# cage-challenge/cage-challenge-4

Hardware: AMD Instinct MI355X
Metric: agent-env steps/sec (5 blue agents x N envs) (higher is better)
Workload: dtype int32

## Files before the change

### cage_challenge_4_amd/csrc/cc4_engine.h

```cpp
#pragma once
#include "cc4_state.h"
#include "cc4_tables.h"

namespace cc4 {

struct Ctx { EnvState* s; EnvCold* c; Rng* r; HostDyn* hd; StepWork* w; unsigned long long* prof = nullptr;
             unsigned long long* aprof = nullptr; EvLog* lg = nullptr; const uint64_t* gpre = nullptr;
             const ExtAct* ext = nullptr; };

#if defined(__HIP_DEVICE_COMPILE__)
#define CC4_TICK(x, i) do { if ((x).prof) { unsigned long long _t = clock64(); (x).prof[(i)] += _t - (x).prof[15]; (x).prof[15] = _t; } } while (0)
#define CC4_TICK0(x) do { if ((x).prof) (x).prof[15] = clock64(); } while (0)
#define CC4_AT0(x) unsigned long long _at = (x).aprof ? clock64() : 0
#define CC4_AT(x, k) do { if ((x).aprof) { unsigned long long _n = clock64(); (x).aprof[(k)] += _n - _at; _at = _n; } } while (0)
#if defined(CC4_FINE)
#define CC4_FT0(x, r) unsigned long long _ft = ((x).aprof && (r) == 0) ? clock64() : 0
#define CC4_FT(x, r, k) do { if ((x).aprof && (r) == 0) { unsigned long long _n = clock64(); (x).aprof[88 + (k)] += _n - _ft; _ft = _n; } } while (0)
#else
#define CC4_FT0(x, r) do { } while (0)
#define CC4_FT(x, r, k) do { } while (0)
#endif
#else
#define CC4_FT0(x, r) do { } while (0)
#define CC4_FT(x, r, k) do { } while (0)
// ... 344 lines not shown
  return r;
}
CC4_HD int rs_kth_on_host(const EnvState* s, const RedAgent& a, int h, int kth) {
  const int n = a.h.nsess;
  for (int i0 = 0; i0 < n; i0 += 8) {
    const S8 q = rs_load8(s, a, i0);
    int hit = -1;
    CC4_UNROLL for (int k = 0; k < 8; ++k)
      if (hit < 0 && i0 + k < n && rsw_host(q.v[k]) == h) { if (kth == 0) hit = i0 + k; kth--; }
    if (hit >= 0) return hit;
  }
  return -1;
}
CC4_HD int rs_find_host_pid(const EnvState* s, const RedAgent& a, int h, int pid) {
  const int n = a.h.nsess;
  for (int i0 = 0; i0 < n; i0 += 8) {
    const S8 q = rs_load8(s, a, i0);
    int hit = -1;
    CC4_UNROLL for (int k = 7; k >= 0; --k) if (i0 + k < n && rsw_host(q.v[k]) == h && rsw_pid(q.v[k]) == pid) hit = i0 + k;
    if (hit >= 0) return hit;
  }
  return -1;
}
struct RedPre { int si = -1; HostSess hs = {0, -1, -1}; bool ok = false; };
#if defined(__HIPCC__)
__device__ __forceinline__ RedPre rs_wave_query(const EnvState* s, int lane, int sid, int host) {
  const int r = lane >> 3, k = lane & 7, ra = r < NRED ? r : 0;
  const RedAgent& A = s->red[ra];
  const int ksid = __builtin_amdgcn_ds_bpermute(ra << 2, sid), khost = __builtin_amdgcn_ds_bpermute(ra << 2, host);
  const int n = (r < NRED && ksid >= 0) ? (int)A.h.nsess : 0;
  const int sh = 8 * k;
  RedPre p; p.ok = true;
  for (int i0 = 0; __ballot(i0 < n); i0 += 8) {
    const bool v = i0 + k < n;
    uint64_t w = 0;
    if (v) w = rs_word(s, A.sord[i0 + k]);
    const bool on = v && rsw_host(w) == khost;
    const uint32_t bid = (uint32_t)(__ballot(v && rsw_id(w) == ksid) >> sh) & 0xFFu;
    const uint32_t bh = (uint32_t)(__ballot(on) >> sh) & 0xFFu, br = (uint32_t)(__ballot(on && (rsw_flags(w) & RS_ROOT)) >> sh) & 0xFFu;
    if (p.si < 0 && bid) p.si = i0 + ctz32(bid);
    p.hs.n += __popc(bh);
    if (p.hs.first < 0 && bh) p.hs.first = i0 + ctz32(bh);
    if (p.hs.first_root < 0 && br) p.hs.first_root = i0 + ctz32(br);
  }
  return p;
}
#endif
CC4_HD void rs_list_remove(RedAgent& a, int idx) {
  uint64_t w[MAX_RS / 8];
  __builtin_memcpy(w, a.sord, MAX_RS);
  const int wi = idx >> 3, sh = 8 * (idx & 7);
  CC4_UNROLL for (int k = 0; k < MAX_RS / 8; ++k) {
    if (k < wi) continue;
    const uint64_t nxt = k + 1 < MAX_RS / 8 ? w[k + 1] : 0ull;
    uint64_t v = (w[k] >> 8) | (nxt << 56);
    if (k == wi && sh) v = (w[k] & ((1ull << sh) - 1ull)) | (v & ~((1ull << sh) - 1ull));
    w[k] = v;
  }
  __builtin_memcpy(a.sord, w, MAX_RS);
}
CC4_HD int rs_alloc_lowest(Ctx x) {
  for (int w = 0; w < RS_POOL / 32; ++w) {
    const uint32_t fr = ~x.s->spool_used[w];
    if (fr) return w * 32 + ctz32(fr);
  }
  return -1;
}
CC4_HD void rs_reserve(Ctx x) {
  uint32_t used[RS_POOL / 32];
  CC4_UNROLL for (int w = 0; w < RS_POOL / 32; ++w) used[w] = x.s->spool_used[w];
  int ty[NRED];
  CC4_UNROLL for (int r = 0; r < NRED; ++r) ty[r] = x.s->rexec[r].type;
  CC4_UNROLL for (int r = 0; r < NRED; ++r) {
    int slot = 0xFF;
    if (ty[r] == RA_EXPLOIT) {
      CC4_UNROLL for (int w = 0; w < RS_POOL / 32; ++w) {
        const uint32_t fr = ~used[w];
        if (slot == 0xFF && fr) { slot = w * 32 + ctz32(fr); used[w] |= 1u << (slot & 31); }
      }
    }
    x.w->rs_slot[r] = (uint8_t)slot;
  }
}
CC4_HD int rs_add(Ctx x, int r, int host, int pid, int flags, int slot = -1) {
  EnvState* s = x.s;
  RedAgent& a = s->red[r];
  if (slot < 0) slot = rs_alloc_lowest(x);
  if (a.h.nsess >= MAX_RS || slot < 0 || slot >= RS_POOL) { set_err(x, E_RSESS_OVERFLOW); return -1; }
  int id = 0;
  for (int i0 = 0; i0 < a.h.nsess; i0 += 8) {
    const S8 q = rs_load8(s, a, i0);
    CC4_UNROLL for (int k = 0; k < 8; ++k) if (i0 + k < a.h.nsess && rsw_id(q.v[k]) + 1 > id) id = rsw_id(q.v[k]) + 1;
  }
  (void)or_shared(&s->spool_used[slot >> 5], 1u << (slot & 31));
  rs_word_put(s, slot, rsw_make(id, pid, host, flags));
  if (flags & RS_ABSTRACT) {
    uint64_t* row = reinterpret_cast<uint64_t*>(x.c->kports[slot]);
    for (int k = 0; k < (MAXH + 7) / 8; ++k) row[k] = 0;
  }
  a.sord[a.h.nsess++] = (uint8_t)slot;
  a.h.rsc_dirty = 1; a.h.fsm_dirty = 1;
  if (!bit_get(a.live_hosts, host)) { bit_set(a.live_hosts, host); a.h.nlive++; }
  bit_set_shared(s->red_hosts, host);
  return a.h.nsess - 1;
}
CC4_HD void rs_host_left(Ctx x, int r, int gone) {
  RedAgent& a = x.s->red[r];
  bit_clr(a.live_hosts, gone); a.h.nlive--;
  uint32_t lw[NRED];
  CC4_UNROLL for (int q = 0; q < NRED; ++q) lw[q] = x.s->red[q].live_hosts[gone >> 5];
  uint32_t any_other = 0;
  CC4_UNROLL for (int q = 0; q < NRED; ++q) any_other |= lw[q];
  if (!((any_other >> (gone & 31)) & 1u)) bit_clr_shared(x.s->red_hosts, gone);
}
CC4_HD void rs_remove_at(Ctx x, int r, int idx, bool keep_record = false) {
  EnvState* s = x.s;
  RedAgent& a = s->red[r];
  const int slot = a.sord[idx];
  const int gone = rsw_host(rs_word(s, slot));
  if (!keep_record) bit_clr_shared(s->spool_used, slot);
  rs_list_remove(a, idx);
  a.h.nsess--;
  a.h.rsc_dirty = 1; a.h.fsm_dirty = 1;
  if (rs_on_host(s, a, gone).n == 0) rs_host_left(x, r, gone);
}
CC4_HD void rs_remove_on_host(Ctx x, int r, int h) {
  EnvState* s = x.s;
  RedAgent& a = s->red[r];
  const int n = a.h.nsess;
  int out = 0, removed = 0;
  bool left = false;
  for (int i0 = 0; i0 < n; i0 += 8) {
    const S8 q = rs_load8(s, a, i0);
    CC4_UNROLL for (int k = 0; k < 8; ++k) {
      if (i0 + k >= n) continue;
      const bool here = rsw_host(q.v[k]) == h;
      if (here && !(rsw_flags(q.v[k]) & RS_ORIG)) { bit_clr_shared(s->spool_used, s8_slot(q, k)); removed++; continue; }
      if (here) left = true;
      if (out != i0 + k) a.sord[out] = (uint8_t)s8_slot(q, k);
      out++;
    }
  }
  if (!removed) return;
  a.h.nsess = (uint8_t)out;
  a.h.rsc_dirty = 1; a.h.fsm_dirty = 1;
  if (!left) rs_host_left(x, r, h);
}
CC4_HD void rs_move_to_end(EnvState* s, RedAgent& a, int idx, int new_id) {
  const int slot = a.sord[idx];
  rs_list_remove(a, idx);
  a.sord[a.h.nsess - 1] = (uint8_t)slot;
  if (new_id >= 0) rs_word_put(s, slot, (rs_word(s, slot) & ~0xFFFFull) | (uint64_t)(new_id & 0xFFFF));
  a.h.rsc_dirty = 1;
}
CC4_HD bool sid_known(const RedAgent& a, const uint16_t* ks, int id, int nknown) {
  if (id < 256) return bit_get(a.known_bm, id);
  for (int i = 0; i < nknown; ++i) if (ks[i] == id) return true;
  return false;
}
CC4_HD void as_know_sid(Ctx x, int r, int id) {
  RedAgent& a = x.s->red[r];
  if (sid_known(a, x.c->known_sid[r], id, a.h.nknown)) return;
  if (a.h.nknown >= MAX_KS) { set_err(x, E_KS_OVERFLOW); return; }
  x.c->known_sid[r][a.h.nknown++] = (uint16_t)id;
  if (id < 256) bit_set(a.known_bm, id);
}
// ... 1258 lines not shown
    }
    if (!bit_get(A.fsm_known, h)) {
      fsm_set_state(A, h, H.fsm_step == 0 ? FS_U : FS_K);
      A.fsm_order[H.fsm_n++] = (uint8_t)h;
      bit_set(A.fsm_known, h);
    }
    if (hn) bit_set(A.fsm_hn, h);
  }
  CC4_AT(x, 4);
  if (H.rsc_listed) {
    const B5 live = b5_load(A.live_hosts), known = b5_load(A.fsm_known), hn = b5_load(A.fsm_hn);
    seen = b5_or(seen, live);
    if (b5_any(b5_andn(live, known)))
      for (int i = 0; i < H.nsess; ++i) {
        int h = rsw_host(rs_at(x.s, A, i));
        if (bit_get(A.fsm_known, h)) continue;
        fsm_set_state(A, h, H.fsm_step == 0 ? FS_U : FS_K);
        A.fsm_order[H.fsm_n++] = (uint8_t)h;
        bit_set(A.fsm_known, h);
      }
    b5_store(A.fsm_hn, b5_or(hn, live));
    H.fsm_dirty = 0;
  }
  CC4_AT(x, 5);
  {
    const B5 lost = b5_andn(b5_load(A.fsm_ur), seen);
    if (b5_any(lost))
      CC4_UNROLL for (int w = 0; w < 5; ++w) {
        uint32_t m = lost.w[w];
        while (m) { int b = ctz32(m); m &= m - 1; fsm_set_state(A, w * 32 + b, FS_KD); }
      }
  }
  CC4_AT(x, 6);
}
CC4_HD int fsm_choose_host_discovery(Ctx x, int r, RedHdr& H) {
  RedAgent& A = x.s->red[r];
  uint32_t order = 0; int nst = 0; uint32_t seen = 0;
  for (int i = 0; i < H.fsm_n && nst < 8; ++i) {
    int st = fsm_get(A, A.fsm_order[i]);
    if (!((seen >> st) & 1u)) { seen |= 1u << st; order |= (uint32_t)st << (4 * nst); nst++; }
  }
  int sum = 0;
  for (int k = 0; k < nst; ++k) { int st = (order >> (4 * k)) & 0xF; sum += st <= FS_SD ? 20 : (st <= FS_UD ? 10 : 0); }
  int chosen_state;
  if (sum > 0) {
    double mult = 1.0 / ((double)sum / 100.0);
    double last = 0.0;
    for (int k = 0; k < nst; ++k) { int st = (order >> (4 * k)) & 0xF; int p = st <= FS_SD ? 20 : (st <= FS_UD ? 10 : 0); last = last + ((double)p / 100.0) * mult; }
    double u = rng_random(x.r);
    double run = 0.0; int idx = 0;
    for (int k = 0; k < nst; ++k) {
      int st = (order >> (4 * k)) & 0xF; int p = st <= FS_SD ? 20 : (st <= FS_UD ? 10 : 0);
      run = run + ((double)p / 100.0) * mult;
      if (run / last <= u) idx++;
    }
    if (idx >= nst) idx = nst - 1;
    chosen_state = (order >> (4 * idx)) & 0xF;
  } else {
    chosen_state = (order >> (4 * (int)rng_below(x.r, (uint32_t)nst))) & 0xF;
  }
  int n_all = 0, n_srv = 0;
  for (int i = 0; i < H.fsm_n; ++i) {
    int h = A.fsm_order[i];
    if (fsm_get(A, h) != chosen_state) continue;
    n_all++;
    if (h_is_server(h) && bit_get(A.fsm_hn, h)) n_srv++;
  }
  int want_srv = -1;
  if (n_all > 1 && n_srv > 0) {
    double i01 = rng_random(x.r);
    want_srv = (i01 <= 0.75 || n_srv == n_all) ? 1 : 0;
  }
  int cnt = want_srv < 0 ? n_all : (want_srv ? n_srv : n_all - n_srv);
  int c = (int)rng_below(x.r, (uint32_t)cnt);
  for (int i = 0; i < H.fsm_n; ++i) {
    int h = A.fsm_order[i];
    if (fsm_get(A, h) != chosen_state) continue;
    bool srv = h_is_server(h) && bit_get(A.fsm_hn, h);
    if (want_srv >= 0 && (int)srv != want_srv) continue;
    if (c-- == 0) return h;
  }
  return A.fsm_order[0];
}
CC4_HD Act fsm_get_action(Ctx x, int r, RedHdr& H, bool observed = false) {
  EnvState* s = x.s;
  RedAgent& A = s->red[r];
  Act out; out.type = RA_SLEEP; out.host = 0; out.arg = 0; out.ticks = 1; out.sid = 0; out.busy = 0;
  CC4_FT0(x, r);
  if (!observed) fsm_observe(x, r, H);
  CC4_FT(x, r, 5);
  if (H.obs_success == T_IN_PROGRESS) { H.fsm_step++; return out; }
  int n = H.fsm_n;
  if (n == 0) { set_err(x, E_FSM_NO_HOST); H.fsm_step++; return out; }
  const bool discovery = (s->policy & 3) == RP_DISCOVERY;
  int host;
  if (!discovery) host = A.fsm_order[rng_below(x.r, (uint32_t)n)];
  else host = fsm_choose_host_discovery(x, r, H);
  CC4_FT(x, r, 6);
  uint32_t pk;
  const int host_state = fsm_get(A, host);
  if (!discovery) switch (host_state) {
    case FS_K:  pk = 0xF432u << 16 | (RA_DRS | RA_AGGR << 4 | RA_STEALTH << 8); break;
    case FS_KD: pk = 0xFF42u << 16 | (RA_AGGR | RA_STEALTH << 4); break;
    case FS_S:  pk = 0xF431u << 16 | (RA_DRS | RA_EXPLOIT << 4 | RA_DECEPTION << 8); break;
    case FS_SD: pk = 0xFF43u << 16 | (RA_EXPLOIT | RA_DECEPTION << 4); break;
    case FS_U:  pk = 0xF442u << 16 | (RA_DRS | RA_PRIVESC << 4 | RA_WITHDRAW << 8); break;
    case FS_UD: pk = 0xFF44u << 16 | (RA_PRIVESC | RA_WITHDRAW << 4); break;
    case FS_R:  pk = 0x4432u << 16 | (RA_DRS | RA_DEGRADE << 4 | RA_IMPACT << 8 | RA_WITHDRAW << 12); break;
    default:    pk = 0xF442u << 16 | (RA_DEGRADE | RA_IMPACT << 4 | RA_WITHDRAW << 8); break;
  } else switch (host_state) {
    case FS_K:  pk = 0xF441u << 16 | (RA_DRS | RA_AGGR << 4 | RA_STEALTH << 8); break;
    case FS_KD: pk = 0xFF44u << 16 | (RA_AGGR | RA_STEALTH << 4); break;
    case FS_S:  pk = 0xF441u << 16 | (RA_DRS | RA_EXPLOIT << 4 | RA_DECEPTION << 8); break;
    case FS_SD: pk = 0xFF44u << 16 | (RA_EXPLOIT | RA_DECEPTION << 4); break;
    case FS_U:  pk = 0xF440u << 16 | (RA_DRS | RA_PRIVESC << 4 | RA_WITHDRAW << 8); break;
    case FS_UD: pk = 0xFF44u << 16 | (RA_PRIVESC | RA_WITHDRAW << 4); break;
    case FS_R:  pk = 0x4444u << 16 | (RA_DRS | RA_DEGRADE << 4 | RA_IMPACT << 8 | RA_WITHDRAW << 12); break;
    default:    pk = 0xF442u << 16 | (RA_DEGRADE | RA_IMPACT << 4 | RA_WITHDRAW << 8); break;
  }
  const int fl = rng_random_quarter(x.r);
  int k = 0;
  for (int i = 0; i < 4; ++i) if ((int)((pk >> (16 + 4 * i)) & 0xF) <= fl) k++;
  int t = (int)((pk >> (4 * k)) & 0xF);
  out.type = (uint8_t)t; out.host = (uint8_t)host;
  bool bad = false;
  if (t == RA_DRS) {
    uint32_t known = H.as_subnet;
    if (known == 0) bad = true; else out.arg = (uint8_t)nth_bit(known, (int)rng_below(x.r, (uint32_t)popc32(known)));
  }
  if ((t == RA_PRIVESC || t == RA_IMPACT || t == RA_DEGRADE) && !bit_get(A.fsm_hn, host)) bad = true;
  if (!bad) {
    if (H.nknown == 0) bad = true; else out.sid = x.c->known_sid[r][rng_below(x.r, (uint32_t)H.nknown)];
  }
  if (bad) { set_err(x, E_UNREACHABLE); out.type = RA_SLEEP; }
  out.ticks = (uint8_t)red_duration(out.type);
  H.fsm_step++;
  CC4_FT(x, r, 7);
  return out;
}
CC4_HD Act random_red_get_action(Ctx x, int r, RedHdr& H) {
  RedAgent& A = x.s->red[r];
  Act out; out.type = RA_SLEEP; out.host = 0; out.arg = 0; out.ticks = 1; out.sid = 0; out.busy = 0;
  const int nip = popc32(A.as_ip[0]) + popc32(A.as_ip[1]) + popc32(A.as_ip[2]) + popc32(A.as_ip[3]) + popc32(A.as_ip[4]);
  const int nhn = popc32(A.as_hn[0]) + popc32(A.as_hn[1]) + popc32(A.as_hn[2]) + popc32(A.as_hn[3]) + popc32(A.as_hn[4]);
  const int nsub = popc32(H.as_subnet), nsid = H.nknown;
  const uint8_t types[10] = {RA_DRS, RA_AGGR, RA_STEALTH, RA_EXPLOIT, RA_PRIVESC, RA_DEGRADE, RA_DECEPTION, RA_IMPACT, RA_WITHDRAW, RA_SLEEP};
  uint32_t valid = 0;
  for (int c = 0; c < 10; ++c) {
    int t = types[c];
    bool ok = true;
    if (t != RA_SLEEP && nsid == 0) ok = false;
    if (t == RA_DRS && nsub == 0) ok = false;
    if ((t == RA_AGGR || t == RA_STEALTH || t == RA_EXPLOIT || t == RA_DECEPTION || t == RA_WITHDRAW) && nip == 0) ok = false;
    if ((t == RA_PRIVESC || t == RA_DEGRADE || t == RA_IMPACT || t == RA_WITHDRAW) && nhn == 0) ok = false;
    if (ok) valid |= 1u << c;
  }
  const int t = types[nth_bit(valid, (int)rng_below(x.r, (uint32_t)popc32(valid)))];
  auto pick_sid = [&]() { return (int)x.c->known_sid[r][rng_below(x.r, (uint32_t)nsid)]; };
  auto pick_ip = [&]() { return nth_set(A.as_ip, 5, (int)rng_below(x.r, (uint32_t)nip)); };
  auto pick_hn = [&]() { return nth_set(A.as_hn, 5, (int)rng_below(x.r, (uint32_t)nhn)); };
  out.type = (uint8_t)t;
  switch (t) {
    case RA_DRS: out.arg = (uint8_t)nth_bit(H.as_subnet, (int)rng_below(x.r, (uint32_t)nsub)); out.sid = (uint16_t)pick_sid(); break;
    case RA_AGGR: case RA_STEALTH: case RA_DECEPTION: out.sid = (uint16_t)pick_sid(); out.host = (uint8_t)pick_ip(); break;
    case RA_EXPLOIT: out.host = (uint8_t)pick_ip(); out.sid = (uint16_t)pick_sid(); break;
    case RA_PRIVESC: case RA_DEGRADE: case RA_IMPACT: out.host = (uint8_t)pick_hn(); out.sid = (uint16_t)pick_sid(); break;
    case RA_WITHDRAW: out.sid = (uint16_t)pick_sid(); out.host = (uint8_t)pick_ip(); out.arg = (uint8_t)pick_hn(); break;
    default: break;
  }
  out.ticks = (uint8_t)red_duration(out.type);
  H.fsm_step++;
  return out;
}
CC4_HD void red_validate(Ctx x, int r, const RedHdr& H, Act& a) {
  RedAgent& A = x.s->red[r];
  if (a.type >= RA_SLEEP) return;
  bool ok = true;
  if (!sid_known(A, x.c->known_sid[r], a.sid, H.nknown)) ok = false;
  if (a.type == RA_DRS) { if (!((H.as_subnet >> a.arg) & 1u)) ok = false; }
  else if (a.type == RA_PRIVESC || a.type == RA_IMPACT || a.type == RA_DEGRADE) { if (!bit_get(A.as_hn, a.host)) ok = false; }
  else if (a.type == RA_WITHDRAW) { if (!bit_get(A.as_ip, a.host) || !bit_get(A.as_hn, a.arg)) ok = false; }
  else { if (!bit_get(A.as_ip, a.host)) ok = false; }
  if (!ok) { a.type = RA_INVALID; a.ticks = 1; }
}

CC4_HD constexpr uint32_t red_zone_hosts(int r, int w) {
  uint32_t m = 0;
  for (int i = 0; i < red_nsub(r); ++i) {
    int lo = red_subnet_alloc(r, i) * SLOTS - 32 * w, hi = lo + SLOTS - 1;
    if (hi < 0 || lo > 31) continue;
    uint32_t up = hi >= 31 ? 0xFFFFFFFFu : ((2u << hi) - 1u);
    uint32_t dn = lo <= 0 ? 0xFFFFFFFFu : (0xFFFFFFFFu << lo);
    m |= up & dn;
  }
  return m;
}
CC4_HD void red_reassign(Ctx x, uint32_t foreign) {
  EnvState* s = x.s;
  uint32_t* mv = x.w->scratch; int nm = 0;
  const int cap = (int)(sizeof(x.w->scratch) / 4);
  for (int r = 0; r < NRED; ++r) {
    if (!((foreign >> r) & 1u)) continue;
// ... 315 lines not shown
    CC4_UNROLL for (int b = a + 1; b < NRED; ++b)
      if (ty[a] >= RA_AGGR && ty[a] <= RA_DEGRADE && ty[b] >= RA_AGGR && ty[b] <= RA_DEGRADE && ho[a] == ho[b]) m |= (1u << a) | (1u << b);
  }
  return withdraw ? (1u << NRED) - 1u : m;
}
CC4_HD uint32_t red_conflict_lane(const EnvState* s, int lane) {
  const int a = lane & 7, b = lane >> 3;
  if (a >= NRED || b >= NRED) return 0u;
  uint32_t va, vb;
  __builtin_memcpy(&va, &s->rexec[a], 4); __builtin_memcpy(&vb, &s->rexec[b], 4);
  const int ta = (int)(va & 0xFF), tb = (int)(vb & 0xFF);
  const bool same = a != b && ta >= RA_AGGR && ta <= RA_DEGRADE && tb >= RA_AGGR && tb <= RA_DEGRADE && ((va ^ vb) & 0xFF00u) == 0;
  return (same ? 1u : 0u) | (ta == RA_WITHDRAW ? 2u : 0u);
}
#if defined(__HIPCC__)
__device__ __forceinline__ uint32_t red_conflict_wave(const EnvState* s, int lane) {
  const uint32_t v = red_conflict_lane(s, lane);
  const uint32_t m = red_foreign_fold(__ballot((v & 1u) != 0));
  return __ballot((v & 2u) != 0) ? (1u << NRED) - 1u : m;
}
#endif
CC4_HD void step_red_exec(Ctx x) {
  rs_reserve(x);
  for (int r = 0; r < NRED; ++r) step_red_exec_agent(x, r);
  step_red_merge(x);
  CC4_TICK(x, 7);
}
CC4_HD void step_reassign(Ctx x, uint32_t foreign) {
  EnvState* s = x.s;
  if (foreign) red_reassign(x, foreign);
  else {
    int ns[NRED];
    CC4_UNROLL for (int r = 0; r < NRED; ++r) ns[r] = s->red[r].h.nsess;
    CC4_UNROLL for (int r = 0; r < NRED; ++r) s->red[r].h.active = (uint8_t)(ns[r] > 0);
  }
  CC4_TICK(x, 8);
}
CC4_HD void red_active_from_sessions(EnvState* s, int r) { s->red[r].h.active = (uint8_t)(s->red[r].h.nsess > 0); }
CC4_HD constexpr uint32_t monitor_watch_mask(int w) {
  uint32_t m = 0;
  for (int i = 0; i < 4; ++i) { const int h = 4 * w + i; if (h < MAXH && ((0xf444f3210ull >> (4 * (h / SLOTS))) & 0xF) != 0xF) m |= 0xFFu << (8 * i); }
  return m;
}
CC4_HD uint32_t monitor_roll4(uint32_t ev4, uint32_t watch) {
  static_assert(EV_OLD_CONN == EV_CUR_CONN << 2 && EV_OLD_PROC == EV_CUR_PROC << 2 && (EV_CUR_CONN | EV_CUR_PROC) == 3, "current bits move up two places");
  return (ev4 & ~watch) | (((ev4 & 0x03030303u) << 2) & watch);
}
CC4_HD uint8_t monitor_roll(int h, uint8_t ev) {
  if (blue_of_subnet(h_subnet(h)) < 0) return ev;
  uint8_t nev = 0;
  if (ev & EV_CUR_CONN) nev |= EV_OLD_CONN;
  if (ev & EV_CUR_PROC) nev |= EV_OLD_PROC;
  return nev;
}
CC4_HD int step_monitor_host(Ctx x, int h) {
  EnvState* s = x.s;
  if (!bit_get(s->exists, h)) return 0;
  const uint8_t ev = s->hev[h];
  const uint8_t nev = monitor_roll(h, ev);
  if (nev != ev) s->hev[h] = nev;
  return nev;
}
CC4_HD void step_monitor_pend(Ctx x) {
  EnvState* s = x.s;
  for (int i = 0; i < s->npend; ++i) {
    int b = blue_of_subnet(h_subnet((int)(s->pend[i] >> 16)));
    if (b < 0) continue;
    BlueAgent& A = s->blue[b];
    if (A.nsus >= cold_sus_cap(s->steps)) set_err(x, E_SUS_OVERFLOW); else { cold_sus(x.c, s->steps, b)[A.nsus++] = s->pend[i]; bit_set(A.sus_hosts, (int)(s->pend[i] >> 16)); }
  }
  s->npend = 0;
}
CC4_HD void step_rsc(Ctx x, int r) {
  if (!x.s->red[r].h.active) return;
  rng_set_stream(x.r, ST_RED_RSC + (uint32_t)r);
  red_session_check(x, r);
}
CC4_HD void step_messages(EnvState* s, const uint8_t* messages, int b) {
  static_assert(MSG_LEN == 8, "a message is one 8-byte word");
  uint64_t w = 0;
  if (messages) for (int i = 0; i < MSG_LEN; ++i) w |= (uint64_t)(messages[b * MSG_LEN + i] ? 1 : 0) << (8 * i);
  __builtin_memcpy(&s->msg[b][0], &w, 8);
}
CC4_HD void step_end(Ctx x, const uint8_t* messages, bool copy_msgs = true) {
  EnvState* s = x.s;
  s->step_count++;
  s->done = (uint8_t)(s->step_count >= s->steps - 1);
  int brm = s->brm;
  int et[NRED], ns[NRED];
  CC4_UNROLL for (int r = 0; r < NRED; ++r) { et[r] = s->red[r].h.exec_type; ns[r] = s->red[r].h.nsess; }
  CC4_UNROLL for (int r = 0; r < NRED; ++r)
    if (et[r] == RA_IMPACT && ns[r] > 0)
      brm += reward_table(s->phase, h_subnet(s->red[r].h.exec_host), RW_RIA);
  s->action_cost = -(float)s->n_restore;
  s->reward = (float)brm + s->action_cost;
  if (x.ext) for (int g = 0; g < s->n_green; ++g) if (x.w->green_act[g] == 3) bit_set_shared(x.c->gfail, g);
  if (copy_msgs) for (int b = 0; b < NBLUE; ++b) step_messages(s, messages, b);
  s->brm = 0; s->n_restore = 0; s->n_actions = NBLUE + s->n_green + NRED;
  rng_park(&s->rng);
}

CC4_HD void env_step(Ctx x, const int32_t* actions, const uint8_t* messages ) {
  EnvState* s = x.s;
  CC4_TICK0(x);
  if (!step_phase(x)) return;
  rng_policy_swap(x, false);
  for (int b = 0; b < NBLUE; ++b) step_blue_submit(x, b, actions ? actions[b] : -1);
  CC4_TICK(x, 0);
  for (int g = 0; g < s->n_green; ++g) step_green_policy(x, g);
  CC4_TICK(x, 1);
  for (int r = 0; r < NRED; ++r) s->n_actions -= step_red_policy_tick(x, r);
  rng_policy_swap(x, true);
  CC4_TICK(x, 2);
  for (int b = 0; b < NBLUE; ++b) step_tick_blue(x, b);
  step_blue_exec(x);
  for (int g = 0; g < s->n_green; ++g) {
    s->brm += step_green_exec(x, g);
    if (bit_get(x.w->phish_mask, g)) { bit_clr(x.w->phish_mask, g); rng_set_stream(x.r, ST_GREEN_PHISH + (uint32_t)g); phishing(x, s->green_host[g]); }
  }
  CC4_TICK(x, 6);
  step_red_exec(x);
  {
    step_reassign(x, red_foreign_agents(s));
  }
  for (int h = 0; h < MAXH; ++h) step_monitor_host(x, h);
  step_monitor_pend(x);
  CC4_TICK(x, 9);
  for (int r = 0; r < NRED; ++r) step_rsc(x, r);
  CC4_TICK(x, 10);
  step_end(x, messages);
}

enum : int { SE_SET_PHASE = 0, SE_ADD_SERVICE = 1, SE_SET_RELIABILITY = 2, SE_CLEAR_HOST = 3, SE_DEPLOY_DECOY = 4, SE_ADD_RED_SESSION = 5,
             SE_BLOCK = 6, SE_SET_STEP = 7, SE_ADD_EVENT = 8, SE_SET_RED_ACTIVE = 9 };
inline int state_edit(Ctx x, int op, int a0, int a1, int a2) {
  EnvState* s = x.s;
  auto host_ok = [&](int h) { return h >= 0 && h < MAXH && bit_get(s->exists, h); };
  switch (op) {
    case SE_SET_PHASE:
      if (a0 < 0 || a0 > 2) return -1;
      s->phase = a0; s->obs_dirty = OD_PHASE;
      return 0;
    case SE_ADD_SERVICE: {
      if (!host_ok(a0) || a1 < K_SSHD || a1 > K_DEC_VSFTPD) return -1;
      HostDyn& d = x.hd[a0];
      const int nsv = hd_nsvc(d);
      int si = -1;
      for (int i = nsv - 1; i >= 0; --i) if (d.svcs[i].kind == a1) si = i;
      if (si < 0 && nsv >= MAXSV) return -1;
      const int pid = create_pid(x, a0);
      if (!add_proc(x, a0, pid, K_PLAIN, a2 ? PF_ROOT : 0)) return -1;
      if (si < 0) { si = nsv; hd_set_nsvc(d, nsv + 1); }
      d.svcs[si].kind = (uint8_t)a1; d.svcs[si].pid = (uint16_t)pid; d.svcs[si].st = (uint8_t)(SV_ACTIVE | 5);
      return pid;
    }
    case SE_SET_RELIABILITY: {
      if (!host_ok(a0) || a1 < 0 || a1 > 100 || a1 % 20) return -1;
      HostDyn& d = x.hd[a0];
      for (int i = 0; i < hd_nsvc(d); ++i) d.svcs[i].st = (uint8_t)((d.svcs[i].st & SV_ACTIVE) | (a1 / 20));
      return 0;
    }
    case SE_CLEAR_HOST: {
      if (!host_ok(a0)) return -1;
      HostDyn& d = x.hd[a0];
      d.nproc = 0; hd_set_nsvc(d, 0);
      for (int i = 0; i < PIN; ++i) { d.procs[i].pid = 0; d.procs[i].kind = 0; d.procs[i].flags = 0; }
      for (int i = 0; i < MAXSV; ++i) { d.svcs[i].pid = 0; d.svcs[i].kind = 0; d.svcs[i].st = 0; }
      return 0;
    }
    case SE_DEPLOY_DECOY: {
      if (!host_ok(a0) || a1 < K_DEC_APACHE || a1 > K_DEC_VSFTPD) return -1;
      HostDyn& d = x.hd[a0];
      const int used = proc_ports(x, a0);
      const int need = a1 == K_DEC_APACHE ? PB_80 : (a1 == K_DEC_TOMCAT ? PB_443 : (a1 == K_DEC_HARAKA ? PB_25 : 0));
      if (used & need) return 0;
      const int pid = create_pid(x, a0);
// ... 144 lines not shown
```

### cage_challenge_4_amd/csrc/cc4_philox1_body.h

```cpp
#pragma once
#include "cc4_kernels.h"

__device__ __forceinline__ void philox1_autoreset(const StepArgs& a, const int e, const int lane, EnvState* s, HostDyn* const hd, EnvCold* const cold_e, StepWork& work) {
    reset_counter_mode_block<WAVE, true>(s, hd, cold_e, &work, lane, a.reset_ws + (size_t)e * RESET_WS_WORDS, 0, true, a.steps, a.policy, a.topo);
    if (lane == 0) { a.reward[e] = s->reward; a.done[e] = s->done; }
    __syncthreads();
}

#ifndef CC4_STOP_IN_FAST
#define CC4_STOP_IN_FAST 0
#endif
#define CC4_STOP_ON (LOG || CC4_STOP_IN_FAST)
#define CC4_STOP(n) do { if (CC4_STOP_ON && a.dbg_stop == (n)) return; } while (0)
template <bool LOG, bool PERSIST>
__device__ __forceinline__ void philox1_body(StepArgs a, const int e, const uint32_t rand_t, const uint32_t item_k, const int lane,
                                             const bool first = true, const bool last = true) {
  extern __shared__ uint4 lds[];
  __shared__ StepWork work;
  __shared__ unsigned long long prof_lds[LOG ? 16 : 1];
  if constexpr (!LOG) a.prof = nullptr;
  (void)item_k;
  EnvCold* const cold_e = cold_at(a.cold, (size_t)e, cold_row_bytes(a.steps));
  unsigned long long t_begin = a.prof ? clock64() : 0;
  const uint4* src = reinterpret_cast<const uint4*>(a.st + e);
// ... 49 lines not shown
      }
      auto bank_fetch = [&](int shift, uint32_t out[4]) {
        const int addr = ((lane + shift) & (WAVE - 1)) << 2;
#pragma unroll
        for (int k = 0; k < 4; ++k) out[k] = (uint32_t)__builtin_amdgcn_ds_bpermute(addr, (int)bank[k]);
      };
      CC4_STOP(2);
      const bool is_red = lane < NRED;
      unsigned long long* ap = (a.prof && is_red) ? a.prof + PROF_SLOTS * (size_t)e + 16 + 8 * lane : nullptr;
      Ctx xr{s, cold_e, &rl, hd, &work, nullptr, ap, lg};
      Ctx xg{s, cold_e, &rl, hd, &work, nullptr, nullptr, lg};
      xr.ext = xt; xg.ext = xt;
      uint32_t pre_rp[4];
      bank_fetch(BK_RPOL, pre_rp);
      const uint32_t brand = (uint32_t)__builtin_amdgcn_ds_bpermute(((lane + BK_BRAND - 8) & (WAVE - 1)) << 2, (int)bank[0]);
      if (is_red) {
        unsigned long long t0 = ap ? clock64() : 0;
        const int dropped = step_red_policy_tick(xr, lane, false, pre_rp);
        if (ap) ap[0] += clock64() - t0;
        if (dropped) atomicSub(&s->n_actions, 1);
      } else if (lane >= 8 && lane < 8 + NBLUE && !(CC4_STOP_ON && a.dbg_stop == 3)) {
        const int b = lane - 8;
        int32_t act = !a.actions ? -1 : a.act_sys ? __hip_atomic_load(a.actions + e * NBLUE + b, __ATOMIC_RELAXED, __HIP_MEMORY_SCOPE_SYSTEM) : a.actions[e * NBLUE + b];
        if (a.rand_out) { act = (int32_t)(((uint64_t)brand * (uint32_t)(b == 4 ? ACT_LONG : ACT_SHORT)) >> 32); a.rand_out[e * NBLUE + b] = act; }
        step_blue_submit(xg, b, act);
        step_tick_blue(xg, b);
        if (!msgs_clean) step_messages(s, a.msgs ? a.msgs + e * NBLUE * MSG_LEN : nullptr, b);
      }
      if (!(CC4_STOP_ON && (a.dbg_stop == 3 || a.dbg_stop == 4))) {
        if (lane < ng) step_green_policy(xg, lane);
        if (lane + WAVE < ng) step_green_policy(xg, lane + WAVE, bank);
      }
      __syncthreads();
      CC4_TICK(x0, 2);
      CC4_STOP(3); CC4_STOP(4); CC4_STOP(5);
      {
        const bool indep = blue_exec_independent(s);
        if (lane == 0) CC4_TICK(x0, 3);
        uint32_t c[4];
        bank_fetch(BK_BEXE, c);
        Ctx xb = xg;
        if (!indep) xb.prof = x0.prof;
        const int rounds = indep ? 1 : 2 * NBLUE;
#pragma nounroll
        for (int i = 0; i < rounds; ++i) {
          int b = lane;
          bool go = lane < NBLUE;
          if (!indep) {
            b = i < NBLUE ? i : i - NBLUE;
            const int ty = s->bexec[b].type;
            go = lane == 0 && ((ty == BA_BLOCK || ty == BA_ALLOW) == (i < NBLUE));
          }
          if (go) {
            rng_set_stream(&rl, ST_BLUE_EXE + (uint32_t)b);
            if (indep) rng_preload(&rl, c);
            blue_execute(xb, b, s->bexec[b]);
          }
        }
        __syncthreads();
        if (lane == 0) CC4_TICK(x0, 5);
      }
      CC4_STOP(6);
      {
        int pen = 0;
        const uint32_t act0 = lane < ng ? work.green_act[lane] : 2u, act1 = lane + WAVE < ng ? work.green_act[lane + WAVE] : 2u;
        const unsigned long long m0 = __ballot(act0 < 2u), m1 = __ballot(act1 < 2u);
        const unsigned long long lt = (1ull << lane) - 1ull;
        const int n0 = __popcll(m0), nact = n0 + __popcll(m1);
        uint8_t* const glist = reinterpret_cast<uint8_t*>(work.scratch);
        static_assert(sizeof(work.scratch) >= MAXG, "the green list fits the scratch words");
        if (act0 < 2u) glist[__popcll(m0 & lt)] = (uint8_t)lane;
        if (act1 < 2u) glist[n0 + __popcll(m1 & lt)] = (uint8_t)(lane + WAVE);
        __syncthreads();
        for (int i = lane; i < nact; i += WAVE) {
          const int g = glist[i];
          uint32_t c[4]; rng_block(&rl, ST_GREEN_EXE + (uint32_t)g, 0, c);
          pen += step_green_exec(xg, g, c);
        }
        if (pen) atomicAdd(&s->brm, pen);
      }
      __syncthreads();
      CC4_TICK(x0, 6);
      CC4_STOP(7);
      if (lane == 0) { step_phishing(x0); CC4_TICK(x0, 1); rs_reserve(x0); }
      __syncthreads();
      const uint32_t serial_red = red_conflict_wave(s, lane);
      if (lane == 0 && prof && serial_red) prof[4] += 1000000;
      CC4_STOP(8);
      uint32_t pre_re[4];
      bank_fetch(BK_REXE, pre_re);
      {
        uint32_t todo = serial_red;
        bool side = true;
#pragma nounroll
        for (;;) {
          int r = lane;
          bool go = is_red && !((serial_red >> lane) & 1u);
          Ctx xe = xr;
          if (!side) { r = __ffs((int)todo) - 1; todo &= todo - 1u; go = lane == 0; xe.prof = x0.prof; xe.aprof = nullptr; }
          RedPre pe;
          if (side) {
            const bool look = go && s->rexec[lane].type < RA_SLEEP;
            pe = rs_wave_query(s, lane, look ? (int)s->rexec[lane].sid : -1, look ? (int)s->rexec[lane].host : -1);
          }
          if (go) {
            unsigned long long t0 = xe.aprof ? clock64() : 0;
            if (s->rexec[r].type != RA_NONE) {
              rng_set_stream(&rl, ST_RED_EXE + (uint32_t)r);
              if (side) rng_preload(&rl, pre_re);
              red_execute(xe, r, s->rexec[r], pe);
            }
            if (xe.aprof) xe.aprof[1] += clock64() - t0;
          }
          __syncthreads();
          side = false;
          if (!todo) break;
        }
      }
      CC4_STOP(9);
      if (lane == 0) { step_red_merge(x0); CC4_TICK(x0, 7); }
      __syncthreads();
      {
        const uint32_t foreign = red_foreign_wave(s, lane);
        if (foreign) { if (lane == 0) red_reassign(x0, foreign); }
        else if (is_red) red_active_from_sessions(s, lane);
        if (lane == 0) CC4_TICK(x0, 8);
      }
      CC4_STOP(10);
      monitor_roll_all(s, lane);
      __syncthreads();
      CC4_TICK(x0, 9);
      CC4_STOP(11);
      if (is_red) { unsigned long long t0 = ap ? clock64() : 0; step_rsc(xr, lane); if (ap) ap[2] += clock64() - t0; }
      if (lane == WAVE - 1) {
        step_monitor_pend(xg);
        step_end(xg, nullptr, false);
        a.reward[e] = s->reward; a.done[e] = s->done;
      }
      CC4_TICK(x0, 10);
    } else if (lane == 0) { a.reward[e] = s->reward; a.done[e] = s->done; }
  }
  __syncthreads();
  CC4_STOP(12);
  unsigned long long t_obs = a.prof ? clock64() : 0;
  {
    int32_t* o = a.obs + (size_t)e * OBS_TOTAL;
    const uint32_t dirty = (do_reset || (a.full_obs && (!PERSIST || item_k == 0))) ? (uint32_t)OD_ALL : (uint32_t)s->obs_dirty;
    encode_obs_fast<WAVE>(s, o, nullptr, false, lane, msgs_clean && !do_reset && dirty != (uint32_t)OD_ALL);
    encode_obs_slow(s, o, dirty, lane);
  }
  __syncthreads();
  CC4_STOP(13);
  if (lane == 0) a.err[e] = s->err;
  unsigned long long t_out = a.prof ? clock64() : 0;
  if (prof && lane == 0) prof[12] += t_out - t_obs;
  if (last) stage_out<HOT_VEC>(reinterpret_cast<uint4*>(a.st + e), lds, lane);
  if (a.obs8) {
    asm volatile("s_waitcnt vmcnt(0)" ::: "memory");
    pack_row_from_obs(a.obs8 + (size_t)e * OBS_PACKED, a.obs + (size_t)e * OBS_TOTAL, lane);
  }
  if (prof && lane == 0) { prof[13] += clock64() - t_out; prof[14] += clock64() - t_begin; }
  if (prof) { __syncthreads(); if (lane < 15) a.prof[PROF_SLOTS * (size_t)e + lane] += prof_lds[lane]; }
}
```

Measured before the change: 1.524 billion.

## Parallelize slot reservation, impact reward and skip idle phishing/merge per wave

Replaces the lane-0 serial rs_reserve with a per-lane computation that ranks each exploiting red agent among free pool bits. Phishing and red-merge now run only when a wave ballot shows pending work. The impact reward term moves from step_end into per-red-lane atomic adds. The FSM action option switch becomes a constexpr lookup table. Together these aim to shorten single-lane serial sections inside the per-env step. The cost is extra ballots, conditional barriers, and a subtle ordering dependence: brm is now updated before step_rsc, and the reservation order must match the serial version.

```diff
diff --git a/cage_challenge_4_amd/csrc/cc4_engine.h b/cage_challenge_4_amd/csrc/cc4_engine.h
--- a/cage_challenge_4_amd/csrc/cc4_engine.h
+++ b/cage_challenge_4_amd/csrc/cc4_engine.h
@@ -450,6 +450,17 @@
     x.w->rs_slot[r] = (uint8_t)slot;
   }
 }
+CC4_HD int rs_reserve_lane(const EnvState* s, uint32_t exploit_mask, int r) {
+  if (!((exploit_mask >> r) & 1u)) return 0xFF;
+  int k = popc32(exploit_mask & ((1u << r) - 1u));
+  int slot = 0xFF;
+  CC4_UNROLL for (int w = 0; w < RS_POOL / 32; ++w) {
+    const uint32_t fr = ~s->spool_used[w];
+    const int c = popc32(fr);
+    if (slot == 0xFF) { if (k < c) slot = w * 32 + nth_bit(fr, k); else k -= c; }
+  }
+  return slot;
+}
 CC4_HD int rs_add(Ctx x, int r, int host, int pid, int flags, int slot = -1) {
   EnvState* s = x.s;
   RedAgent& a = s->red[r];
@@ -1874,6 +1885,49 @@
   }
   return A.fsm_order[0];
 }
+CC4_HD constexpr uint32_t fsm_pk_switch(bool discovery, int host_state) {
+  if (!discovery) switch (host_state) {
+    case FS_K:  return 0xF432u << 16 | (RA_DRS | RA_AGGR << 4 | RA_STEALTH << 8);
+    case FS_KD: return 0xFF42u << 16 | (RA_AGGR | RA_STEALTH << 4);
+    case FS_S:  return 0xF431u << 16 | (RA_DRS | RA_EXPLOIT << 4 | RA_DECEPTION << 8);
+    case FS_SD: return 0xFF43u << 16 | (RA_EXPLOIT | RA_DECEPTION << 4);
+    case FS_U:  return 0xF442u << 16 | (RA_DRS | RA_PRIVESC << 4 | RA_WITHDRAW << 8);
+    case FS_UD: return 0xFF44u << 16 | (RA_PRIVESC | RA_WITHDRAW << 4);
+    case FS_R:  return 0x4432u << 16 | (RA_DRS | RA_DEGRADE << 4 | RA_IMPACT << 8 | RA_WITHDRAW << 12);
+    default:    return 0xF442u << 16 | (RA_DEGRADE | RA_IMPACT << 4 | RA_WITHDRAW << 8);
+  } else switch (host_state) {
+    case FS_K:  return 0xF441u << 16 | (RA_DRS | RA_AGGR << 4 | RA_STEALTH << 8);
+    case FS_KD: return 0xFF44u << 16 | (RA_AGGR | RA_STEALTH << 4);
+    case FS_S:  return 0xF441u << 16 | (RA_DRS | RA_EXPLOIT << 4 | RA_DECEPTION << 8);
+    case FS_SD: return 0xFF44u << 16 | (RA_EXPLOIT | RA_DECEPTION << 4);
+    case FS_U:  return 0xF440u << 16 | (RA_DRS | RA_PRIVESC << 4 | RA_WITHDRAW << 8);
+    case FS_UD: return 0xFF44u << 16 | (RA_PRIVESC | RA_WITHDRAW << 4);
+    case FS_R:  return 0x4444u << 16 | (RA_DRS | RA_DEGRADE << 4 | RA_IMPACT << 8 | RA_WITHDRAW << 12);
+    default:    return 0xF442u << 16 | (RA_DEGRADE | RA_IMPACT << 4 | RA_WITHDRAW << 8);
+  }
+}
+struct FsmPkTab { uint32_t v[16]; };
+CC4_HD constexpr int fsm_pk_index(bool discovery, int host_state) { return (discovery ? 8 : 0) + (host_state < 7 ? host_state : 7); }
+constexpr FsmPkTab make_fsm_pk_tab() {
+  FsmPkTab t{};
+  for (int d = 0; d < 2; ++d) for (int st = 0; st < 8; ++st) t.v[fsm_pk_index(d != 0, st)] = fsm_pk_switch(d != 0, st);
+  return t;
+}
+constexpr bool fsm_pk_tab_matches() {
+  const FsmPkTab t = make_fsm_pk_tab();
+  for (int d = 0; d < 2; ++d) {
+    for (int st = 0; st <= FS_F; ++st) if (t.v[fsm_pk_index(d != 0, st)] != fsm_pk_switch(d != 0, st)) return false;
+    if (t.v[fsm_pk_index(d != 0, FS_NONE)] != fsm_pk_switch(d != 0, FS_NONE)) return false;
+  }
+  return true;
+}
+static_assert(fsm_pk_tab_matches(), "fsm_get_action's option table == its switch");
+#if defined(__HIP_DEVICE_COMPILE__)
+static __device__ const FsmPkTab fsm_pk_tab = make_fsm_pk_tab();
+#else
+static constexpr FsmPkTab fsm_pk_tab = make_fsm_pk_tab();
+#endif
+CC4_HD uint32_t fsm_pk(bool discovery, int host_state) { return fsm_pk_tab.v[fsm_pk_index(discovery, host_state)]; }
 CC4_HD Act fsm_get_action(Ctx x, int r, RedHdr& H, bool observed = false) {
   EnvState* s = x.s;
   RedAgent& A = s->red[r];
@@ -1889,27 +1943,7 @@
   if (!discovery) host = A.fsm_order[rng_below(x.r, (uint32_t)n)];
   else host = fsm_choose_host_discovery(x, r, H);
   CC4_FT(x, r, 6);
-  uint32_t pk;
-  const int host_state = fsm_get(A, host);
-  if (!discovery) switch (host_state) {
-    case FS_K:  pk = 0xF432u << 16 | (RA_DRS | RA_AGGR << 4 | RA_STEALTH << 8); break;
-    case FS_KD: pk = 0xFF42u << 16 | (RA_AGGR | RA_STEALTH << 4); break;
-    case FS_S:  pk = 0xF431u << 16 | (RA_DRS | RA_EXPLOIT << 4 | RA_DECEPTION << 8); break;
-    case FS_SD: pk = 0xFF43u << 16 | (RA_EXPLOIT | RA_DECEPTION << 4); break;
-    case FS_U:  pk = 0xF442u << 16 | (RA_DRS | RA_PRIVESC << 4 | RA_WITHDRAW << 8); break;
-    case FS_UD: pk = 0xFF44u << 16 | (RA_PRIVESC | RA_WITHDRAW << 4); break;
-    case FS_R:  pk = 0x4432u << 16 | (RA_DRS | RA_DEGRADE << 4 | RA_IMPACT << 8 | RA_WITHDRAW << 12); break;
-    default:    pk = 0xF442u << 16 | (RA_DEGRADE | RA_IMPACT << 4 | RA_WITHDRAW << 8); break;
-  } else switch (host_state) {
-    case FS_K:  pk = 0xF441u << 16 | (RA_DRS | RA_AGGR << 4 | RA_STEALTH << 8); break;
-    case FS_KD: pk = 0xFF44u << 16 | (RA_AGGR | RA_STEALTH << 4); break;
-    case FS_S:  pk = 0xF441u << 16 | (RA_DRS | RA_EXPLOIT << 4 | RA_DECEPTION << 8); break;
-    case FS_SD: pk = 0xFF44u << 16 | (RA_EXPLOIT | RA_DECEPTION << 4); break;
-    case FS_U:  pk = 0xF440u << 16 | (RA_DRS | RA_PRIVESC << 4 | RA_WITHDRAW << 8); break;
-    case FS_UD: pk = 0xFF44u << 16 | (RA_PRIVESC | RA_WITHDRAW << 4); break;
-    case FS_R:  pk = 0x4444u << 16 | (RA_DRS | RA_DEGRADE << 4 | RA_IMPACT << 8 | RA_WITHDRAW << 12); break;
-    default:    pk = 0xF442u << 16 | (RA_DEGRADE | RA_IMPACT << 4 | RA_WITHDRAW << 8); break;
-  }
+  const uint32_t pk = fsm_pk(discovery, fsm_get(A, host));
   const int fl = rng_random_quarter(x.r);
   int k = 0;
   for (int i = 0; i < 4; ++i) if ((int)((pk >> (16 + 4 * i)) & 0xF) <= fl) k++;
@@ -2391,16 +2425,22 @@
   if (messages) for (int i = 0; i < MSG_LEN; ++i) w |= (uint64_t)(messages[b * MSG_LEN + i] ? 1 : 0) << (8 * i);
   __builtin_memcpy(&s->msg[b][0], &w, 8);
 }
-CC4_HD void step_end(Ctx x, const uint8_t* messages, bool copy_msgs = true) {
+CC4_HD int step_impact_term(const EnvState* s, int r) {
+  const RedHdr& h = s->red[r].h;
+  return (h.exec_type == RA_IMPACT && h.nsess > 0) ? reward_table(s->phase, h_subnet(h.exec_host), RW_RIA) : 0;
+}
+CC4_HD void step_end(Ctx x, const uint8_t* messages, bool copy_msgs = true, bool impact = true) {
   EnvState* s = x.s;
   s->step_count++;
   s->done = (uint8_t)(s->step_count >= s->steps - 1);
   int brm = s->brm;
-  int et[NRED], ns[NRED];
-  CC4_UNROLL for (int r = 0; r < NRED; ++r) { et[r] = s->red[r].h.exec_type; ns[r] = s->red[r].h.nsess; }
-  CC4_UNROLL for (int r = 0; r < NRED; ++r)
-    if (et[r] == RA_IMPACT && ns[r] > 0)
-      brm += reward_table(s->phase, h_subnet(s->red[r].h.exec_host), RW_RIA);
+  if (impact) {
+    int et[NRED], ns[NRED];
+    CC4_UNROLL for (int r = 0; r < NRED; ++r) { et[r] = s->red[r].h.exec_type; ns[r] = s->red[r].h.nsess; }
+    CC4_UNROLL for (int r = 0; r < NRED; ++r)
+      if (et[r] == RA_IMPACT && ns[r] > 0)
+        brm += reward_table(s->phase, h_subnet(s->red[r].h.exec_host), RW_RIA);
+  }
   s->action_cost = -(float)s->n_restore;
   s->reward = (float)brm + s->action_cost;
   if (x.ext) for (int g = 0; g < s->n_green; ++g) if (x.w->green_act[g] == 3) bit_set_shared(x.c->gfail, g);
diff --git a/cage_challenge_4_amd/csrc/cc4_philox1_body.h b/cage_challenge_4_amd/csrc/cc4_philox1_body.h
--- a/cage_challenge_4_amd/csrc/cc4_philox1_body.h
+++ b/cage_challenge_4_amd/csrc/cc4_philox1_body.h
@@ -155,7 +155,13 @@
       __syncthreads();
       CC4_TICK(x0, 6);
       CC4_STOP(7);
-      if (lane == 0) { step_phishing(x0); CC4_TICK(x0, 1); rs_reserve(x0); }
+      {
+        const bool phish = __ballot(lane < 3 && work.phish_mask[lane] != 0) != 0ull;
+        const uint32_t exploit = (uint32_t)__ballot(is_red && s->rexec[lane].type == RA_EXPLOIT);
+        if (phish) { if (lane == 0) step_phishing(x0); __syncthreads(); }
+        if (lane == 0) CC4_TICK(x0, 1);
+        if (is_red) work.rs_slot[lane] = (uint8_t)(exploit ? rs_reserve_lane(s, exploit, lane) : 0xFF);
+      }
       __syncthreads();
       const uint32_t serial_red = red_conflict_wave(s, lane);
       if (lane == 0 && prof && serial_red) prof[4] += 1000000;
@@ -191,13 +197,15 @@
         }
       }
       CC4_STOP(9);
-      if (lane == 0) { step_red_merge(x0); CC4_TICK(x0, 7); }
+      if (__ballot(is_red && work.pend_r[lane] != 0)) { if (lane == 0) step_red_merge(x0); }
+      if (lane == 0) CC4_TICK(x0, 7);
       __syncthreads();
       {
         const uint32_t foreign = red_foreign_wave(s, lane);
-        if (foreign) { if (lane == 0) red_reassign(x0, foreign); }
+        if (foreign) { if (lane == 0) red_reassign(x0, foreign); __syncthreads(); }
         else if (is_red) red_active_from_sessions(s, lane);
         if (lane == 0) CC4_TICK(x0, 8);
+        if (is_red) { const int term = step_impact_term(s, lane); if (term) atomicAdd(&s->brm, term); }
       }
       CC4_STOP(10);
       monitor_roll_all(s, lane);
@@ -207,7 +215,7 @@
       if (is_red) { unsigned long long t0 = ap ? clock64() : 0; step_rsc(xr, lane); if (ap) ap[2] += clock64() - t0; }
       if (lane == WAVE - 1) {
         step_monitor_pend(xg);
-        step_end(xg, nullptr, false);
+        step_end(xg, nullptr, false, false);
         a.reward[e] = s->reward; a.done[e] = s->done;
       }
       CC4_TICK(x0, 10);
```

New measurement: 1.576 billion (median of 6 runs). +3.4%, better.
